# 86885974647565434342125458569795756674/torch.distributed.pipeline.sync.Pipe

Measured on AMD Instinct MI355X. Metric: tokens/sec for 12-layer Transformer at PP=N (pipeline-parallel training), higher is better.
Workload: dtype bf16

## Files before the change

mipipe/csrc/kernels/gemm.hip:

```cpp
#include <algorithm>
#include <cstdlib>

#include "common.h"
#include "kernels.h"

namespace mipipe {

namespace {

constexpr int BM = 128, BN = 128, BK = 64;
constexpr int kThreads = 256;
constexpr int kTileBytes = BM * BK * 2;
constexpr int kBufBytes = 2 * kTileBytes;
constexpr int kSmemBytes = 2 * kBufBytes;

typedef __attribute__((ext_vector_type(4))) short s16x4;
typedef __attribute__((ext_vector_type(8))) short s16x8;
typedef __attribute__((address_space(3))) s16x4 lds_s16x4;

__device__ __forceinline__ int kc_off(int r, int c16) { return r * 128 + ((c16 ^ ((r >> 1) & 7)) << 4); }

__device__ __forceinline__ int ic_rk(int r) { return (r & 3) | (((r >> 3) & 1) << 2); }
__device__ __forceinline__ int ic_off(int r, int c8) { return r * 256 + ((c8 ^ (ic_rk(r) << 2)) << 3); }

typedef __attribute__((ext_vector_type(4))) unsigned int u32x4;

template <bool KC>
struct Stager {
  u32x4 v[4];
  __device__ __forceinline__ void load(const bf16_t* __restrict__ base, int64_t ld, int i0, int k0, int tid) {
#pragma unroll
    for (int u = 0; u < 4; ++u) {
      const int id = tid + u * kThreads;
      const bf16_t* p;
      if (KC) {
        const int r = id >> 3, c = id & 7;
        p = base + (int64_t)(i0 + r) * ld + k0 + c * 8;
      } else {
        const int r = id >> 4, c = id & 15;
        p = base + (int64_t)(k0 + r) * ld + i0 + c * 8;
      }
      v[u] = *reinterpret_cast<const u32x4*>(p);
    }
  }
  __device__ __forceinline__ void store(char* tile, int tid) const {
#pragma unroll
    for (int u = 0; u < 4; ++u) {
      const int id = tid + u * kThreads;
      int off;
      if (KC) {
        off = kc_off(id >> 3, id & 7);
      } else {
        off = ic_off(id >> 4, (id & 15) * 2);
      }
      *reinterpret_cast<u32x4*>(tile + off) = v[u];
    }
  }
};

template <bool KC>
__device__ __forceinline__ bf16x8 read_frag(const char* tile, int ib, int s, int lane) {
  if (KC) {
    const int r = ib + (lane & 15);
    const int c = 4 * s + (lane >> 4);
    return *reinterpret_cast<const bf16x8*>(tile + kc_off(r, c));
  } else {
    const int g = lane >> 4, q = (lane & 15) >> 2, p = lane & 3;
    const int r0 = 32 * s + 8 * g + q;
    const int c8 = (ib >> 2) + p;
    const s16x4 lo = __builtin_amdgcn_ds_read_tr16_b64_v4i16((lds_s16x4*)(tile + ic_off(r0, c8)));
    const s16x4 hi = __builtin_amdgcn_ds_read_tr16_b64_v4i16((lds_s16x4*)(tile + ic_off(r0 + 4, c8)));
    const s16x8 both = __builtin_shufflevector(lo, hi, 0, 1, 2, 3, 4, 5, 6, 7);
    return __builtin_bit_cast(bf16x8, both);
  }
}

__device__ __forceinline__ float dact_f(int dact, float s) {
  return dact == kActRelu ? (s > 0.f ? 1.f : 0.f) : (dact == kActSavedGrad ? s : gelu_grad_f(s));
}

__device__ __forceinline__ void tile_coords(int tiles_m, int tiles_n, int& tm, int& tn, int G = 8) {
  const int nwg = tiles_m * tiles_n;
  const int bid = blockIdx.x;
  int wg = bid;
  if (nwg > 8) {
    const int xcd = bid & 7, local = bid >> 3;
    const int q = nwg >> 3, r = nwg & 7;
    wg = (xcd < r ? xcd * (q + 1) : r * (q + 1) + (xcd - r) * q) + local;
  }
  const int group = wg / (G * tiles_n);
  const int first_m = group * G;
  const int gsize = min(tiles_m - first_m, G);
  const int in_group = wg % (G * tiles_n);
  tm = first_m + in_group % gsize;
  tn = in_group / gsize;
}

template <bool A_KC, bool B_KC, int EPI, int ACT>
__global__ void __launch_bounds__(kThreads) gemm_kernel(GemmArgs g) {
  extern __shared__ __attribute__((aligned(16))) char smem[];
  const int tid = threadIdx.x;
  const int lane = tid & 63;
  const int wave = tid >> 6;
  const int wm = wave >> 1, wn = wave & 1;

  int tm, tn;
  tile_coords(g.M / BM, g.N / BN, tm, tn);
  const int m0 = tm * BM, n0 = tn * BN;

  const bf16_t* A = reinterpret_cast<const bf16_t*>(g.A);
  const bf16_t* B = reinterpret_cast<const bf16_t*>(g.B);

  f32x4 acc[4][4];
#pragma unroll
  for (int i = 0; i < 4; ++i)
#pragma unroll
    for (int j = 0; j < 4; ++j) acc[i][j] = f32x4{0.f, 0.f, 0.f, 0.f};

  Stager<A_KC> sa;
  Stager<B_KC> sb;
  const int nk = g.K / BK;

  sa.load(A, g.lda, m0, 0, tid);
  sb.load(B, g.ldb, n0, 0, tid);
  sa.store(smem, tid);
  sb.store(smem + kTileBytes, tid);
  __syncthreads();

  for (int kt = 0; kt < nk; ++kt) {
    char* cur = smem + (kt & 1) * kBufBytes;
    const bool more = kt + 1 < nk;
    if (more) {
      sa.load(A, g.lda, m0, (kt + 1) * BK, tid);
      sb.load(B, g.ldb, n0, (kt + 1) * BK, tid);
    }
#pragma unroll
    for (int s = 0; s < 2; ++s) {
      bf16x8 af[4], bfr[4];
#pragma unroll
      for (int t = 0; t < 4; ++t) af[t] = read_frag<A_KC>(cur, wm * 64 + 16 * t, s, lane);
#pragma unroll
      for (int t = 0; t < 4; ++t) bfr[t] = read_frag<B_KC>(cur + kTileBytes, wn * 64 + 16 * t, s, lane);
#pragma unroll
      for (int i = 0; i < 4; ++i)
#pragma unroll
        for (int j = 0; j < 4; ++j) acc[i][j] = __builtin_amdgcn_mfma_f32_16x16x32_bf16(af[i], bfr[j], acc[i][j], 0, 0, 0);
    }
    if (more) {
      char* nxt = smem + ((kt + 1) & 1) * kBufBytes;
      sa.store(nxt, tid);
      sb.store(nxt + kTileBytes, tid);
    }
    __syncthreads();
  }

  const int quad = lane >> 4, col_in = lane & 15;
  const float pscale = g.p > 0.f ? 1.f / (1.f - g.p) : 1.f;
#pragma unroll
  for (int i = 0; i < 4; ++i) {
    const int row0 = m0 + wm * 64 + 16 * i + 4 * quad;
#pragma unroll
    for (int j = 0; j < 4; ++j) {
      const int col = n0 + wn * 64 + 16 * j + col_in;
      f32x4 v = acc[i][j];
      if (EPI == kEpiAccumF32) {
        float* C = reinterpret_cast<float*>(g.C);
#pragma unroll
        for (int r = 0; r < 4; ++r) {
          float* p = C + (int64_t)(row0 + r) * g.ldc + col;
          *p += v[r];
        }
      } else if (EPI == kEpiStoreF32) {
        float* C = reinterpret_cast<float*>(g.C);
#pragma unroll
        for (int r = 0; r < 4; ++r) C[(int64_t)(row0 + r) * g.ldc + col] = v[r];
      } else {
        bf16_t* C = reinterpret_cast<bf16_t*>(g.C);
        const float b = g.bias != nullptr ? bf2f(reinterpret_cast<const bf16_t*>(g.bias)[col]) : 0.f;
        float pre[4], out[4];
#pragma unroll
        for (int r = 0; r < 4; ++r) {
          pre[r] = v[r] + b;
          out[r] = ACT == kActRelu ? fmaxf(pre[r], 0.f) : (ACT == kActGelu ? gelu_f(pre[r]) : pre[r]);
        }
        if (g.p > 0.f) {
          const uint4 w = Philox(g.seed, drop_sub(row0, col, g.N), g.offset).next4();
          const uint32_t ws[4] = {w.x, w.y, w.z, w.w};
#pragma unroll
          for (int r = 0; r < 4; ++r) out[r] = drop_keep(ws[r], col & 1, g.threshold >> 16) ? out[r] * pscale : 0.f;
        }
#pragma unroll
        for (int r = 0; r < 4; ++r) {
          if (g.dact_in != nullptr && g.dact == kActReluBits)
            out[r] *= (reinterpret_cast<const uint8_t*>(g.dact_in)[(int64_t)(row0 + r) * g.ldd + (col >> 3)] >> (col & 7)) & 1
                          ? g.dact_scale : 0.f;
          else if (g.dact_in != nullptr)
            out[r] *= g.dact_scale *
                      dact_f(g.dact, bf2f(reinterpret_cast<const bf16_t*>(g.dact_in)[(int64_t)(row0 + r) * g.ldd + col]));
          if (g.res != nullptr) out[r] += bf2f(reinterpret_cast<const bf16_t*>(g.res)[(int64_t)(row0 + r) * g.ldr + col]);
          C[(int64_t)(row0 + r) * g.ldc + col] = f2bf(out[r]);
          if (g.aux != nullptr)
            reinterpret_cast<bf16_t*>(g.aux)[(int64_t)(row0 + r) * g.ldc + col] =
                f2bf(g.aux_grad ? gelu_grad_f(pre[r]) : pre[r]);
        }
      }
    }
  }
}

namespace big {

constexpr int BM = 256, BN = 256, BK = 64;
constexpr int kThreads = 512;
constexpr int kTileBytes = BM * BK * 2;
constexpr int kSmemBytes = 128 * 260 * 4;

template <bool B_KC, int W>
constexpr int smem_bytes() {
  constexpr int b3 = 2 * (kTileBytes + W * BK * 2) + W * BK * 2;
  return !B_KC && b3 > kSmemBytes ? b3 : kSmemBytes;
}

template <int W>
__device__ __forceinline__ int ic_off_w(int r, int c8) { return r * (2 * W) + ((c8 ^ (ic_rk(r) << 2)) << 3); }

template <bool KC, int W>
__device__ __forceinline__ void stage_offsets(int64_t ld, int i0, int lim, int wave, int lane, uint32_t (&off)[W / 64]) {
  constexpr int NU = W / 64, LPR = W / 8;
#pragma unroll
  for (int u = 0; u < NU; ++u) {
    const int inst = wave * NU + u;
    if (KC) {
      const int row = 8 * inst + (lane >> 3);
      const int c = (lane & 7) ^ ((row >> 1) & 7);
      const int gi = min(i0 + row, lim - 1);
      off[u] = (uint32_t)(((int64_t)gi * ld + 8 * c) * 2);
    } else {
      const int row = (64 / LPR) * inst + lane / LPR;
      const int c16 = (lane % LPR) ^ (ic_rk(row) << 1);
      const int gi = min(i0 + 8 * c16, lim - 8);
      off[u] = (uint32_t)(((int64_t)row * ld + gi) * 2);
    }
  }
}

__device__ __forceinline__ void stage_offsets_halves(int64_t ld, int i0, int lim, int share, int lane,
                                                     uint32_t (&off)[4]) {
  const int half = share >> 2;
#pragma unroll
  for (int u = 0; u < 4; ++u) {
    const int row = 4 * (4 * (share & 3) + u) + (lane >> 4);
    const int c16 = (lane & 15) ^ (ic_rk(row) << 1);
    const int gi = min(i0 + 128 * half + 8 * c16, lim - 8);
    off[u] = (uint32_t)(((int64_t)row * ld + gi) * 2);
  }
}

__device__ __forceinline__ void glds16_saddr(const char* base, uint32_t off, const char* lds_dst) {
  const uint32_t m0 = (uint32_t)(uintptr_t)((__attribute__((address_space(3))) const char*)lds_dst);
  asm volatile(
      "s_mov_b32 m0, %0\n\t"
      "s_nop 0\n\t"
      "global_load_lds_dwordx4 %1, %2"
      :
      : "s"(m0), "v"(off), "s"(base)
      : "memory", "m0");
}

template <int N>
__device__ __forceinline__ void vmcnt_keep() {
  asm volatile("s_waitcnt vmcnt(%0)" ::"n"(N) : "memory");
}

constexpr int kWaitLgkm0 = 0xC07F;

template <int W>
__device__ __forceinline__ void stage_fast(const char* base, const uint32_t (&off)[W / 64], char* tile, int wave) {
  constexpr int NU = W / 64;
#pragma unroll
  for (int u = 0; u < NU; ++u) glds16_saddr(base, off[u], tile + (wave * NU + u) * 1024);
}

struct KCursor {
  const char *a, *b;
  const char *na, *nb;
  int64_t step_a, step_b;
  int seg_k, kl, seg;

  __device__ __forceinline__ void load_next(const GemmArgs& g) {
    const int nx = min(seg + 1, GemmArgs::kMaxSegs - 1);
    na = reinterpret_cast<const char*>(g.a_seg[nx]);
    nb = reinterpret_cast<const char*>(g.b_seg[nx]);
  }
  template <bool A_KC, bool B_KC>
  __device__ __forceinline__ void init(const GemmArgs& g, int kt) {
    const int64_t lda = g.lda, ldb = g.ldb;
    step_a = A_KC ? BK * 2 : BK * lda * 2;
    step_b = B_KC ? BK * 2 : BK * ldb * 2;
    seg_k = g.seg_k;
    kl = kt * BK;
    seg = 0;
    a = na = reinterpret_cast<const char*>(g.A);
    b = nb = reinterpret_cast<const char*>(g.B);
    if (seg_k > 0) {
      seg = kl / seg_k;
      kl -= seg * seg_k;
      a = reinterpret_cast<const char*>(g.a_seg[seg]);
      b = reinterpret_cast<const char*>(g.b_seg[seg]);
      load_next(g);
    }
    a += A_KC ? (int64_t)kl * 2 : (int64_t)kl * lda * 2;
    b += B_KC ? (int64_t)kl * 2 : (int64_t)kl * ldb * 2;
  }
  __device__ __forceinline__ void next(const GemmArgs& g) {
    a += step_a;
    b += step_b;
    kl += BK;
    if (__builtin_expect(kl == seg_k, 0)) {
      kl = 0;
      ++seg;
      a = na;
      b = nb;
      load_next(g);
    }
  }
};

template <bool KC, int W>
__device__ __forceinline__ bf16x8 frag(const char* tile, int ib, int s, int lane) {
  if (KC) {
    const int r = ib + (lane & 15);
    const int c = 4 * s + (lane >> 4);
    return *reinterpret_cast<const bf16x8*>(tile + kc_off(r, c));
  } else {
    const int g = lane >> 4, q = (lane & 15) >> 2, p = lane & 3;
    const int r0 = 32 * s + 8 * g + q;
    const int c8 = (ib >> 2) + p;
    const s16x4 lo = __builtin_amdgcn_ds_read_tr16_b64_v4i16((lds_s16x4*)(tile + ic_off_w<W>(r0, c8)));
    const s16x4 hi = __builtin_amdgcn_ds_read_tr16_b64_v4i16((lds_s16x4*)(tile + ic_off_w<W>(r0 + 4, c8)));
    return __builtin_bit_cast(bf16x8, __builtin_shufflevector(lo, hi, 0, 1, 2, 3, 4, 5, 6, 7));
  }
}

struct EpiParams {
  uint64_t seed, offset;
  int N;
  float p, pscale;
  uint32_t threshold;
  int mask_row0, mask_col0, mask_ld;
};

template <int I, int ACT, int NJ, bool EXTRA>
__device__ __forceinline__ void epi_rows(const EpiParams ep, f32x4 (&acc)[8][NJ], int nrow, int ncol,
                                         const float (&bias)[NJ]) {
  if constexpr (!EXTRA) {
#pragma unroll
    for (int j = 0; j < NJ; ++j)
#pragma unroll
      for (int r = 0; r < 4; ++r) {
        const float pre = acc[I][j][r] + bias[j];
        acc[I][j][r] = ACT == kActRelu ? fmaxf(pre, 0.f) : (ACT == kActGelu ? gelu_f(pre) : pre);
      }
    return;
  }
  const int row0 = nrow + 16 * I;
#pragma unroll
  for (int j = 0; j < NJ; ++j) {
    const int col = ncol + 16 * j;
    const float b = bias[j];
    uint32_t ws[4] = {0xFFFFFFFFu, 0xFFFFFFFFu, 0xFFFFFFFFu, 0xFFFFFFFFu};
    if (ep.p > 0.f) {
      const uint4 w = Philox(ep.seed, drop_sub(row0 + ep.mask_row0, col + ep.mask_col0, ep.mask_ld), ep.offset).next4();
      ws[0] = w.x; ws[1] = w.y; ws[2] = w.z; ws[3] = w.w;
    }
#pragma unroll
    for (int r = 0; r < 4; ++r) {
      const float pre = acc[I][j][r] + b;
      float out = ACT == kActRelu ? fmaxf(pre, 0.f) : (ACT == kActGelu ? gelu_f(pre) : pre);
      if (ep.p > 0.f) out = drop_keep(ws[r], (col + ep.mask_col0) & 1, ep.threshold >> 16) ? out * ep.pscale : 0.f;
      acc[I][j][r] = out;
    }
  }
}

template <int EPI, int W>
__device__ __forceinline__ void staged_store(char* smem, const f32x4 (&acc)[8][W / 64], int wm, int wn, int lane,
                                             int tid, int m0, int n0, int M, int N, int64_t ldc, void* out,
                                             const bf16_t* res, int64_t ldr = 0, const bf16_t* dact_in = nullptr,
                                             int64_t ldd = 0, int dact = 0, float dact_scale = 1.f,
                                             bool trans = false, bool dgelu = false) {
  constexpr int NJ = W / 64, WN = 16 * NJ, kStride = W + 4;
  const int quad = lane >> 4, col_in = lane & 15;
  float* stg = reinterpret_cast<float*>(smem);
#pragma unroll
  for (int pass = 0; pass < 2; ++pass) {
    if (wm == pass) {
#pragma unroll
      for (int i = 0; i < 8; ++i)
#pragma unroll
        for (int j = 0; j < NJ; ++j)
#pragma unroll
          for (int r = 0; r < 4; ++r)
            stg[(16 * i + 4 * quad + r) * kStride + wn * WN + 16 * j + col_in] = acc[i][j][r];
    }
    __syncthreads();
    const int rbase = m0 + pass * 128;
    auto grow = [&](int R) { return rbase + R; };
    if (EPI == kEpiStoreBf16) {
      bf16_t* C = reinterpret_cast<bf16_t*>(out);
      constexpr int CPR = W / 8;
#pragma unroll
      for (int u = 0; u < 128 * CPR / kThreads; ++u) {
        const int idx = tid + u * kThreads;
        const int row = idx / CPR, c8 = idx % CPR;
        if (grow(row) >= M || n0 + 8 * c8 >= N) continue;
        const f32x4 lo = *reinterpret_cast<const f32x4*>(stg + row * kStride + 8 * c8);
        const f32x4 hi = *reinterpret_cast<const f32x4*>(stg + row * kStride + 8 * c8 + 4);
        const int64_t at = (int64_t)grow(row) * ldc + n0 + 8 * c8;
        float v[8] = {lo[0], lo[1], lo[2], lo[3], hi[0], hi[1], hi[2], hi[3]};
        if (dgelu) {
#pragma unroll
          for (int e = 0; e < 8; ++e) v[e] = gelu_grad_f(v[e]);
        }
        if (dact_in != nullptr && dact == kActReluBits) {
          const uint32_t mb =
              reinterpret_cast<const uint8_t*>(dact_in)[(int64_t)grow(row) * ldd + ((n0 + 8 * c8) >> 3)];
#pragma unroll
          for (int e = 0; e < 8; ++e) v[e] *= (mb >> e) & 1 ? dact_scale : 0.f;
        } else if (dact_in != nullptr) {
          const bf16x8 sv = *reinterpret_cast<const bf16x8*>(dact_in + (int64_t)grow(row) * ldd + n0 + 8 * c8);
#pragma unroll
          for (int e = 0; e < 8; ++e) v[e] *= dact_scale * dact_f(dact, (float)sv[e]);
        }
        if (res != nullptr) {
          const bf16x8 rv = *reinterpret_cast<const bf16x8*>(res + (int64_t)grow(row) * ldr + n0 + 8 * c8);
#pragma unroll
          for (int e = 0; e < 8; ++e) v[e] += (float)rv[e];
        }
        bf16x8 o;
#pragma unroll
        for (int e = 0; e < 8; ++e) o[e] = (__bf16)v[e];
        *reinterpret_cast<bf16x8*>(C + at) = o;
      }
    } else if (trans) {
      float* C = reinterpret_cast<float*>(out);
#pragma unroll 4
      for (int u = 0; u < 32 * W / kThreads; ++u) {
        const int idx = tid + u * kThreads;
        const int mq = (idx & 7) + 8 * (idx / (8 * W)), n = (idx >> 3) % W;
        if (grow(4 * mq) >= M || n0 + n >= N) continue;
        const float* sp = stg + 4 * mq * kStride + n;
        const float4 v = make_float4(sp[0], sp[kStride], sp[2 * kStride], sp[3 * kStride]);
        float4* dst = reinterpret_cast<float4*>(C + (int64_t)(n0 + n) * ldc + grow(4 * mq));
        if (EPI == kEpiAccumF32) {
          const float4 o = *dst;
          *dst = make_float4(o.x + v.x, o.y + v.y, o.z + v.z, o.w + v.w);
        } else {
          *dst = v;
        }
      }
    } else {
      float* C = reinterpret_cast<float*>(out);
      constexpr int CPR = W / 4;
#pragma unroll
      for (int u = 0; u < 128 * CPR / kThreads; ++u) {
        const int idx = tid + u * kThreads;
        const int row = idx / CPR, c4 = idx % CPR;
        if (grow(row) >= M || n0 + 4 * c4 >= N) continue;
        const float4 v = *reinterpret_cast<const float4*>(stg + row * kStride + 4 * c4);
        float4* dst = reinterpret_cast<float4*>(C + (int64_t)grow(row) * ldc + n0 + 4 * c4);
        if (EPI == kEpiAccumF32) {
          const float4 o = *dst;
          *dst = make_float4(o.x + v.x, o.y + v.y, o.z + v.z, o.w + v.w);
        } else {
          *dst = v;
        }
      }
    }
    __syncthreads();
  }
}

template <int ACT, int W>
__device__ __forceinline__ void staged_store_act(char* smem, const f32x4 (&acc)[8][W / 64], int wm, int wn,
                                                 int lane, int tid, int m0, int n0, const GemmArgs& g) {
  constexpr int NJ = W / 64, WN = 16 * NJ, kStride = W + 4, CB = W / 8;
  const int quad = lane >> 4, col_in = lane & 15;
  float* stg = reinterpret_cast<float*>(smem);
  bf16_t* C = reinterpret_cast<bf16_t*>(g.C);
  bf16_t* aux = reinterpret_cast<bf16_t*>(g.aux);
  const bf16_t* res = reinterpret_cast<const bf16_t*>(g.res);
  const bf16_t* dact_in = reinterpret_cast<const bf16_t*>(g.dact_in);
  const int64_t ldr = g.ldr > 0 ? g.ldr : g.ldc;
  const bool drop = g.p > 0.f;
  const float pscale = drop ? 1.f / (1.f - g.p) : 1.f;
  const int64_t mask_ld = g.mask_ld > 0 ? g.mask_ld : g.N;
  const uint32_t thr16 = g.threshold >> 16;
#pragma unroll
  for (int pass = 0; pass < 2; ++pass) {
    if (wm == pass) {
#pragma unroll
      for (int i = 0; i < 8; ++i)
#pragma unroll
        for (int j = 0; j < NJ; ++j)
#pragma unroll
          for (int r = 0; r < 4; ++r)
            stg[(16 * i + 4 * quad + r) * kStride + wn * WN + 16 * j + col_in] = acc[i][j][r];
    }
    __syncthreads();
    const int rbase = m0 + pass * 128;
#pragma unroll
    for (int u = 0; u < 32 * CB / kThreads; ++u) {
      const int idx = tid + u * kThreads;
      const int rq = idx / CB, c8 = idx % CB;
      const int col = n0 + 8 * c8;
      const int row0 = rbase + 4 * rq;
      if (col >= g.N || row0 >= g.M) continue;
      uint32_t wd[4][4];
      if (drop) {
        const uint64_t sub = drop_sub(row0 + g.mask_row0, col + g.mask_col0, mask_ld);
#pragma unroll
        for (int e = 0; e < 4; ++e) {
          const uint4 w = Philox(g.seed, sub + e, g.offset).next4();
          wd[e][0] = w.x; wd[e][1] = w.y; wd[e][2] = w.z; wd[e][3] = w.w;
        }
      }
#pragma unroll
      for (int r = 0; r < 4; ++r) {
        const int row = row0 + r;
        if (row >= g.M) break;
        const float* sp = stg + (4 * rq + r) * kStride + 8 * c8;
        const f32x4 lo = *reinterpret_cast<const f32x4*>(sp);
        const f32x4 hi = *reinterpret_cast<const f32x4*>(sp + 4);
        const float pre[8] = {lo[0], lo[1], lo[2], lo[3], hi[0], hi[1], hi[2], hi[3]};
        if (aux != nullptr) {
          bf16x8 a;
#pragma unroll
          for (int e = 0; e < 8; ++e) a[e] = (__bf16)(ACT == kActGelu && g.aux_grad ? gelu_grad_f(pre[e]) : pre[e]);
          *reinterpret_cast<bf16x8*>(aux + (int64_t)row * g.ldc + col) = a;
        }
        float v[8];
#pragma unroll
        for (int e = 0; e < 8; ++e) {
          float o = ACT == kActRelu ? fmaxf(pre[e], 0.f) : (ACT == kActGelu ? gelu_f(pre[e]) : pre[e]);
          if (drop) o = drop_keep(wd[e >> 1][r], e & 1, thr16) ? o * pscale : 0.f;
          v[e] = o;
        }
        if (dact_in != nullptr) {
          const bf16x8 sv = *reinterpret_cast<const bf16x8*>(dact_in + (int64_t)row * g.ldd + col);
#pragma unroll
          for (int e = 0; e < 8; ++e) v[e] *= g.dact_scale * dact_f(g.dact, (float)sv[e]);
        }
        if (res != nullptr) {
          const bf16x8 rv = *reinterpret_cast<const bf16x8*>(res + (int64_t)row * ldr + col);
#pragma unroll
          for (int e = 0; e < 8; ++e) v[e] += (float)rv[e];
        }
        bf16x8 o;
#pragma unroll
        for (int e = 0; e < 8; ++e) o[e] = (__bf16)v[e];
        *reinterpret_cast<bf16x8*>(C + (int64_t)row * g.ldc + col) = o;
        if (g.bits != nullptr) {
          uint32_t mb = 0;
#pragma unroll
          for (int e = 0; e < 8; ++e) mb |= (v[e] != 0.f ? 1u : 0u) << e;
          reinterpret_cast<uint8_t*>(g.bits)[(int64_t)row * g.ldbits + (col >> 3)] = (uint8_t)mb;
        }
      }
    }
    __syncthreads();
  }
}


constexpr int kXEmit = 1, kXColsum = 2;

template <bool A_KC, bool B_KC, int EPI, int ACT, int W, bool EXTRA, int X = 0>
__global__ void __launch_bounds__(kThreads, 1) gemm256_kernel(GemmArgs g) {
  constexpr int NJ = W / 64;
  constexpr int WN = W / 4;
  constexpr int kBuf = kTileBytes + W * BK * 2;
  constexpr bool AH = !A_KC;
  constexpr bool B3 = !B_KC;
  extern __shared__ __attribute__((aligned(16))) char smem[];
  const int tid = threadIdx.x;
  const int lane = tid & 63;
  const int wave = __builtin_amdgcn_readfirstlane(tid >> 6);
  const int wm = wave >> 2, wn = wave & 3;

  int tm, tn;
  tile_coords((g.M + BM - 1) / BM, (g.N + W - 1) / W, tm, tn, g.group_m);
  tm = __builtin_amdgcn_readfirstlane(tm);
  tn = __builtin_amdgcn_readfirstlane(tn);
  const int m0 = tm * BM, n0 = tn * W;
  f32x4 acc[8][NJ];
#pragma unroll
  for (int i = 0; i < 8; ++i)
#pragma unroll
    for (int j = 0; j < NJ; ++j) acc[i][j] = f32x4{0.f, 0.f, 0.f, 0.f};

  const bool rsum = g.rowsum != nullptr && tn < 16 && !A_KC;
  float rs[4] = {0.f, 0.f, 0.f, 0.f};
  auto rowsum_read = [&](const char* tile, s16x4& v) {
    if (rsum && wm == 0) {
      const int r = tid >> 2, c8 = 4 * tn + (tid & 3);
      v = *reinterpret_cast<const s16x4*>(
          AH ? tile + (tn >> 3) * (kTileBytes / 2) + ic_off_w<128>(r, c8 & 31) : tile + ic_off_w<256>(r, c8));
    }
  };
  auto rowsum_add = [&](const s16x4& v) {
    if (rsum && wm == 0) {
#pragma unroll
      for (int e = 0; e < 4; ++e) rs[e] += __uint_as_float((uint32_t)(uint16_t)v[e] << 16);
    }
  };
  const int tiles_m = (g.M + BM - 1) / BM;
  const int cm_log = __builtin_amdgcn_readfirstlane(2 * tiles_m * 16 >= W ? 0 : 2 * tiles_m * 32 >= W ? 1
                                                    : 2 * tiles_m * 64 >= W ? 2 : 3);
  const int csl = tm + tiles_m * wm;
  const bool csum = X == kXColsum && !B_KC && g.colsum != nullptr && csl < (W / 16 >> cm_log);
  float cs[4] = {0.f, 0.f, 0.f, 0.f};
  auto colsum_step = [&](const char* btile) {
    if (csum) {
      const int t = tid & 255;
      const int q = t & ((4 << cm_log) - 1), r0 = t >> (2 + cm_log);
      for (int j = 0; j < (1 << cm_log); ++j) {
        const s16x4 v = *reinterpret_cast<const s16x4*>(
            btile + ic_off_w<W>(r0 + (j << (6 - cm_log)), (4 << cm_log) * csl + q));
#pragma unroll
        for (int e = 0; e < 4; ++e) cs[e] += __uint_as_float((uint32_t)(uint16_t)v[e] << 16);
      }
    }
  };
  const int ntn = (g.N + W - 1) / W;
  const int ewb = __builtin_amdgcn_readfirstlane((4 * wave) % ntn);
  auto emit_reads = [&](const char* atile, int j, s16x4& a, s16x4& b) {
    const int q = (lane & 15) >> 2, p = lane & 3, gq = lane >> 4;
    const int c16 = 2 * gq + (p >> 1);
    const int r = 8 * (4 * wave + j) + q;
    const int lo = r * 128 + ((c16 ^ ((r >> 1) & 7)) << 4) + 8 * (p & 1);
    const int hi = (r + 4) * 128 + ((c16 ^ (((r + 4) >> 1) & 7)) << 4) + 8 * (p & 1);
    a = __builtin_amdgcn_ds_read_tr16_b64_v4i16((lds_s16x4*)(atile + lo));
    b = __builtin_amdgcn_ds_read_tr16_b64_v4i16((lds_s16x4*)(atile + hi));
  };
  bf16_t* const at_out = X == kXEmit ? reinterpret_cast<bf16_t*>(g.at) : nullptr;
  const int64_t ldat = X == kXEmit ? g.ldat : 0;
  const int M = g.M;
  auto emit_store = [&](int kt, int j, const s16x4& a, const s16x4& b) {
    const int rb = 4 * wave + j;
    bf16_t* at = at_out + (int64_t)(kt * BK + 16 * (lane >> 4) + (lane & 15)) * ldat + m0 + 8 * rb;
    if (m0 + 8 * rb < M) *reinterpret_cast<s16x8*>(at) = __builtin_shufflevector(a, b, 0, 1, 2, 3, 4, 5, 6, 7);
  };
  int kt0 = 0, nk = g.K / BK;
  if (g.k_splits > 1) {
    const int total = nk;
    kt0 = (int)blockIdx.y * total / g.k_splits;
    nk = ((int)blockIdx.y + 1) * total / g.k_splits - kt0;
  }
  const int shA = wave ^ 4;
  const int shB = B_KC ? 2 * wn + (wm == 0 ? 1 : 0) : wave;
  uint32_t offA[4], offB[NJ];
  if constexpr (AH) stage_offsets_halves(g.lda, m0, g.M, shA, lane, offA);
  else stage_offsets<A_KC, 256>(g.lda, m0, g.M, shA, lane, offA);
  stage_offsets<B_KC, W>(g.ldb, n0, g.N, shB, lane, offB);
  constexpr int NB = W / 64;
  constexpr int NA = 4;
  KCursor kc;
  kc.init<A_KC, B_KC>(g, kt0);
  stage_fast<256>(kc.a, offA, smem, shA);
  stage_fast<W>(kc.b, offB, smem + kTileBytes, shB);
  kc.next(g);
  if (wm == 1 && nk > 1) {
    stage_fast<256>(kc.a, offA, smem + kBuf, shA);
    stage_fast<W>(kc.b, offB, smem + kBuf + kTileBytes, shB);
    kc.next(g);
  }

  if (wm == 1 && nk > 1) vmcnt_keep<NA + NB>();
  else asm volatile("s_waitcnt vmcnt(0)" ::: "memory");
  __builtin_amdgcn_s_barrier();
  if (wm == 1) __builtin_amdgcn_s_barrier();
  bf16x8 af[8][2], bq[NJ][2];
  int ekt = kt0 % ntn;
  auto bslot = [&](int s) { return s == 2 ? smem + 2 * kBuf : smem + s * kBuf + kTileBytes; };
  int bs = 0;
  for (int u = 0; u < nk; ++u) {
    char* cur = smem + (u & 1) * kBuf;
    char* nxt = smem + ((u + 1) & 1) * kBuf;
    char* bcur = B3 ? bslot(bs) : cur + kTileBytes;
    int ej = -1;
    if (X == kXEmit && A_KC) {
      int e = ewb + ekt;
      while (e >= ntn) e -= ntn;
      ej = tn - e;
      if (ej < 0) ej += ntn;
      if (ntn < 4) {
        for (int j = ej; j < 4; j += ntn) {
          s16x4 a, b;
          emit_reads(cur, j, a, b);
          emit_store(kt0 + u, j, a, b);
        }
        ej = -1;
      } else if (ej > 3) {
        ej = -1;
      }
    }
    s16x4 ea, eb;
    if (X == kXEmit && A_KC && ej >= 0) emit_reads(cur, ej, ea, eb);
#pragma unroll
    for (int ii = 0; ii < 8; ++ii)
#pragma unroll
      for (int s = 0; s < 2; ++s)
        af[ii][s] = AH ? frag<false, 128>(cur + wm * (kTileBytes / 2), 16 * ii, s, lane)
                       : frag<A_KC, 256>(cur, wm * 128 + 16 * ii, s, lane);
#pragma unroll
    for (int j = 0; j < NJ; ++j)
#pragma unroll
      for (int s = 0; s < 2; ++s) bq[j][s] = frag<B_KC, W>(bcur, wn * WN + 16 * j, s, lane);
    s16x4 rv;
    rowsum_read(cur, rv);
    if (X == kXEmit && A_KC && ej >= 0) emit_store(kt0 + u, ej, ea, eb);
    ekt = ekt + 1 == ntn ? 0 : ekt + 1;
    const int ahead = wm == 0 ? 1 : 2;
    if (u + ahead < nk) {
      char* dst = wm == 0 ? nxt : cur;
      stage_fast<256>(kc.a, offA, dst, shA);
      int bn = bs + ahead;
      if (bn >= 3) bn -= 3;
      stage_fast<W>(kc.b, offB, B3 ? bslot(bn) : dst + kTileBytes, shB);
      kc.next(g);
    }
    bs = bs == 2 ? 0 : bs + 1;
    colsum_step(bcur);
    if (wm == 1) {
      if (u + 2 < nk) vmcnt_keep<NA + NB>();
      else asm volatile("s_waitcnt vmcnt(0)" ::: "memory");
    }
    __builtin_amdgcn_s_waitcnt(kWaitLgkm0);
    rowsum_add(rv);
    __builtin_amdgcn_sched_barrier(0);
    __builtin_amdgcn_s_barrier();
    __builtin_amdgcn_sched_barrier(0);
    __builtin_amdgcn_s_setprio(1);
#pragma unroll
    for (int s = 0; s < 2; ++s)
#pragma unroll
      for (int ii = 0; ii < 8; ++ii)
#pragma unroll
        for (int j = 0; j < NJ; ++j)
          acc[ii][j] = __builtin_amdgcn_mfma_f32_16x16x32_bf16(af[ii][s], bq[j][s], acc[ii][j], 0, 0, 0);
    __builtin_amdgcn_s_setprio(0);
    if (wm == 0) asm volatile("s_waitcnt vmcnt(0)" ::: "memory");
    __builtin_amdgcn_sched_barrier(0);
    __builtin_amdgcn_s_barrier();
    __builtin_amdgcn_sched_barrier(0);
  }
  if (wm == 0) __builtin_amdgcn_s_barrier();

  if (rsum) {
    __syncthreads();
    float* red = reinterpret_cast<float*>(smem);
    if (wm == 0) {
#pragma unroll
      for (int e = 0; e < 4; ++e)
#pragma unroll
        for (int o = 4; o < 64; o <<= 1) rs[e] += __shfl_xor(rs[e], o, 64);
      if (lane < 4)
#pragma unroll
        for (int e = 0; e < 4; ++e) red[wave * 16 + 4 * lane + e] = rs[e];
    }
    __syncthreads();
    if (tid < 16) {
      const float v = red[tid] + red[16 + tid] + red[32 + tid] + red[48 + tid];
      const int row = m0 + 16 * tn + tid;
      if (row < g.M) g.rowsum[row] += v;
    }
  }
  if (X == kXColsum && g.colsum != nullptr) {
    __syncthreads();
    const int sw = 16 << cm_log;
    float* red = reinterpret_cast<float*>(smem) + 64;
#pragma unroll
    for (int e = 0; e < 4; ++e)
      for (int o = 4 << cm_log; o < 64; o <<= 1) cs[e] += __shfl_xor(cs[e], o, 64);
    if (lane < (4 << cm_log))
#pragma unroll
      for (int e = 0; e < 4; ++e) red[wave * sw + 4 * lane + e] = cs[e];
    __syncthreads();
    if (tid < 2 * sw) {
      const int gq = tid >> (4 + cm_log), c = tid & (sw - 1);
      const int sl = tm + tiles_m * gq;
      float v = 0.f;
#pragma unroll
      for (int w = 0; w < 4; ++w) v += red[(4 * gq + w) * sw + c];
      const int col = n0 + sw * sl + c;
      if (sl < (W / 16 >> cm_log) && col < g.N) {
        if (g.k_splits > 1) g.colsum[(int64_t)blockIdx.y * g.N + col] = v;
        else g.colsum[col] += v;
      }
    }
  }
  const int quad = lane >> 4, col_in = lane & 15;
  __syncthreads();
  if (EPI == kEpiStoreBf16 && EXTRA) {
    const int ncol = n0 + wn * WN + col_in;
    if (g.bias != nullptr) {
#pragma unroll
      for (int j = 0; j < NJ; ++j) {
        const float b = ncol + 16 * j < g.N ? bf2f(reinterpret_cast<const bf16_t*>(g.bias)[ncol + 16 * j]) : 0.f;
#pragma unroll
        for (int i = 0; i < 8; ++i) acc[i][j] += b;
      }
    }
    staged_store_act<ACT, W>(smem, acc, wm, wn, lane, tid, m0, n0, g);
    return;
  }
  if (EPI == kEpiStoreBf16 && (ACT != kActNone || g.bias != nullptr)) {
    const int ncol = n0 + wn * WN + col_in, nrow = m0 + wm * 128 + 4 * quad;
    const float pscale = g.p > 0.f ? 1.f / (1.f - g.p) : 1.f;
    const EpiParams ep{g.seed, g.offset, g.N, g.p, pscale, g.threshold, g.mask_row0, g.mask_col0,
                       g.mask_ld > 0 ? g.mask_ld : g.N};
    float bias[NJ];
#pragma unroll
    for (int j = 0; j < NJ; ++j)
      bias[j] = (g.bias != nullptr && ncol + 16 * j < g.N) ? bf2f(reinterpret_cast<const bf16_t*>(g.bias)[ncol + 16 * j]) : 0.f;
    epi_rows<0, ACT, NJ, EXTRA>(ep, acc, nrow, ncol, bias);
    epi_rows<1, ACT, NJ, EXTRA>(ep, acc, nrow, ncol, bias);
    epi_rows<2, ACT, NJ, EXTRA>(ep, acc, nrow, ncol, bias);
    epi_rows<3, ACT, NJ, EXTRA>(ep, acc, nrow, ncol, bias);
    epi_rows<4, ACT, NJ, EXTRA>(ep, acc, nrow, ncol, bias);
    epi_rows<5, ACT, NJ, EXTRA>(ep, acc, nrow, ncol, bias);
    epi_rows<6, ACT, NJ, EXTRA>(ep, acc, nrow, ncol, bias);
    epi_rows<7, ACT, NJ, EXTRA>(ep, acc, nrow, ncol, bias);
  }
  void* out = EPI == kEpiStoreBf16 ? g.C
                                   : reinterpret_cast<void*>(reinterpret_cast<float*>(g.C) +
                                                             (int64_t)blockIdx.y * g.M * g.ldc);
  if (EPI == kEpiStoreBf16 && g.dact_in != nullptr)
    staged_store<EPI, W>(smem, acc, wm, wn, lane, tid, m0, n0, g.M, g.N, g.ldc, out,
                         reinterpret_cast<const bf16_t*>(g.res), g.ldr, reinterpret_cast<const bf16_t*>(g.dact_in),
                         g.ldd, g.dact, g.dact_scale);
  else if (EPI != kEpiStoreBf16 && g.trans_c && g.k_splits <= 1)
    staged_store<EPI, W>(smem, acc, wm, wn, lane, tid, m0, n0, g.M, g.N, g.ldc, out, nullptr, 0, nullptr, 0, 0, 1.f,
                         true);
  else
    staged_store<EPI, W>(smem, acc, wm, wn, lane, tid, m0, n0, g.M, g.N, g.ldc, out,
                         EPI == kEpiStoreBf16 ? reinterpret_cast<const bf16_t*>(g.res) : nullptr, g.ldr);
}

}

int big_tiles(const GemmArgs& g, int w) { return ((g.M + big::BM - 1) / big::BM) * ((g.N + w - 1) / w); }

bool use_big(const GemmArgs& g) {
  return g.round_chunk || g.seg_k > 0 || g.at != nullptr || g.trans_c || g.colsum != nullptr || g.rowsum != nullptr ||
         g.M % BM != 0 || g.N % BN != 0 || big_tiles(g, 256) >= 128;
}

int g_gemm_width = -1;
int g_gemm_rounds = -1;

int big_width(const GemmArgs& g) {
  if (g_gemm_width < 0) {
    const char* e = getenv("MIPIPE_GEMM_W");
    g_gemm_width = e ? atoi(e) : 0;
  }
  if (g_gemm_width == 128 || g_gemm_width == 256) return g_gemm_width;
  if (g.width == 128 || g.width == 256) return g.width;
  if (g.k_splits > 1) return 256;
  const int r256 = (big_tiles(g, 256) + 255) / 256, r128 = (big_tiles(g, 128) + 255) / 256;
  return 0.75 * r128 < 1.0 * r256 ? 128 : 256;
}

template <bool A_KC, bool B_KC, int EPI, int ACT, int W, bool EXTRA, int X = 0>
void launch_big(const GemmArgs& g, hipStream_t s) {
  constexpr int smem = big::smem_bytes<B_KC, W>();
  static bool attr_set = false;
  if (!attr_set) {
    (void)hipFuncSetAttribute(
        reinterpret_cast<const void*>(&big::gemm256_kernel<A_KC, B_KC, EPI, ACT, W, EXTRA, X>),
        hipFuncAttributeMaxDynamicSharedMemorySize, smem);
    attr_set = true;
  }
  hipLaunchKernelGGL((big::gemm256_kernel<A_KC, B_KC, EPI, ACT, W, EXTRA, X>), dim3(big_tiles(g, W), g.k_splits),
                     dim3(big::kThreads), smem, s, g);
}

template <bool A_KC, bool B_KC, int EPI, int ACT, bool EXTRA>
void launch_big_w(const GemmArgs& g, hipStream_t s) {
  const bool narrow = big_width(g) == 128;
  if constexpr (A_KC && B_KC && EPI == kEpiStoreBf16 && !(ACT == kActGelu && EXTRA)) {
    if (g.at != nullptr) {
      if (narrow) launch_big<A_KC, B_KC, EPI, ACT, 128, EXTRA, big::kXEmit>(g, s);
      else launch_big<A_KC, B_KC, EPI, ACT, 256, EXTRA, big::kXEmit>(g, s);
      return;
    }
  }
  if constexpr (A_KC && !B_KC && EPI != kEpiStoreBf16 && !EXTRA) {
    if (g.colsum != nullptr) {
      if (narrow) launch_big<A_KC, B_KC, EPI, ACT, 128, EXTRA, big::kXColsum>(g, s);
      else launch_big<A_KC, B_KC, EPI, ACT, 256, EXTRA, big::kXColsum>(g, s);
      return;
    }
  }
  if (narrow) launch_big<A_KC, B_KC, EPI, ACT, 128, EXTRA>(g, s);
  else launch_big<A_KC, B_KC, EPI, ACT, 256, EXTRA>(g, s);
}

int g_gemm_group = -1;

template <bool A_KC, bool B_KC, int EPI, int ACT>
void launch(const GemmArgs& gi, hipStream_t s) {
  if (g_gemm_group < 0) {
    const char* e = getenv("MIPIPE_GEMM_G");
    g_gemm_group = e ? atoi(e) : 0;
  }
  GemmArgs g = gi;
  if (g_gemm_group > 0) g.group_m = g_gemm_group;
  if (use_big(g)) {
    if constexpr (EPI == kEpiStoreBf16) {
      if (g.p > 0.f || g.aux != nullptr) {
        launch_big_w<A_KC, B_KC, EPI, ACT, true>(g, s);
        return;
      }
    }
    launch_big_w<A_KC, B_KC, EPI, ACT, false>(g, s);
    return;
  }
  const int blocks = (g.M / BM) * (g.N / BN);
  hipLaunchKernelGGL((gemm_kernel<A_KC, B_KC, EPI, ACT>), dim3(blocks), dim3(kThreads), kSmemBytes, s, g);
}

__global__ void __launch_bounds__(256) splitk_reduce_kernel(const float* __restrict__ ws, int splits, int M, int N,
                                                            int64_t ldc, const bf16_t* __restrict__ res, int64_t ldr,
                                                            bf16_t* __restrict__ C) {
  const int64_t chunks = (int64_t)M * (N / 8);
  const int64_t c = (int64_t)blockIdx.x * blockDim.x + threadIdx.x;
  if (c >= chunks) return;
  const int row = (int)(c / (N / 8)), col = (int)(c % (N / 8)) * 8;
  const int64_t at = (int64_t)row * N + col;
  f32x4 lo = *reinterpret_cast<const f32x4*>(ws + at);
  f32x4 hi = *reinterpret_cast<const f32x4*>(ws + at + 4);
  for (int s = 1; s < splits; ++s) {
    lo += *reinterpret_cast<const f32x4*>(ws + (int64_t)s * M * N + at);
    hi += *reinterpret_cast<const f32x4*>(ws + (int64_t)s * M * N + at + 4);
  }
  float v[8] = {lo[0], lo[1], lo[2], lo[3], hi[0], hi[1], hi[2], hi[3]};
  const int64_t out = (int64_t)row * ldc + col;
  if (res != nullptr) {
    const bf16x8 r = *reinterpret_cast<const bf16x8*>(res + (int64_t)row * ldr + col);
#pragma unroll
    for (int e = 0; e < 8; ++e) v[e] += (float)r[e];
  }
  bf16x8 o;
#pragma unroll
  for (int e = 0; e < 8; ++e) o[e] = (__bf16)v[e];
  *reinterpret_cast<bf16x8*>(C + out) = o;
}

__global__ void __launch_bounds__(256) splitk_reduce_f32_kernel(const float* __restrict__ ws, int splits, int M, int N,
                                                                int64_t ldc, bool accumulate, bool trans,
                                                                float* __restrict__ C) {
  const int64_t c = (int64_t)blockIdx.x * blockDim.x + threadIdx.x;
  if (trans) {
    if (c >= (int64_t)(M / 4) * N) return;
    const int m = (int)(c / N) * 4, n = (int)(c % N);
    f32x4 v = {0.f, 0.f, 0.f, 0.f};
    for (int s = 0; s < splits; ++s) {
      const float* p = ws + (int64_t)s * M * N + (int64_t)m * N + n;
      v += f32x4{p[0], p[N], p[2 * (int64_t)N], p[3 * (int64_t)N]};
    }
    f32x4* dst = reinterpret_cast<f32x4*>(C + (int64_t)n * ldc + m);
    if (accumulate) v += *dst;
    *dst = v;
    return;
  }
  const int64_t chunks = (int64_t)M * (N / 4);
  if (c >= chunks) return;
  const int row = (int)(c / (N / 4)), col = (int)(c % (N / 4)) * 4;
  const int64_t at = (int64_t)row * N + col;
  f32x4 v = *reinterpret_cast<const f32x4*>(ws + at);
  for (int s = 1; s < splits; ++s) v += *reinterpret_cast<const f32x4*>(ws + (int64_t)s * M * N + at);
  f32x4* dst = reinterpret_cast<f32x4*>(C + (int64_t)row * ldc + col);
  if (accumulate) v += *dst;
  *dst = v;
}

__global__ void __launch_bounds__(256) colsum_splits_kernel(const float* __restrict__ ws, int splits, int N,
                                                            float* __restrict__ colsum) {
  const int n = blockIdx.x * blockDim.x + threadIdx.x;
  if (n >= N) return;
  float v = 0.f;
  for (int s = 0; s < splits; ++s) v += ws[(int64_t)s * N + n];
  colsum[n] += v;
}

int g_gemm_splitk = -1;

template <bool A_KC, bool B_KC, int EPI>
void launch_act(const GemmArgs& g, hipStream_t s) {
  switch (g.act) {
    case kActRelu: launch<A_KC, B_KC, EPI, kActRelu>(g, s); break;
    case kActGelu: launch<A_KC, B_KC, EPI, kActGelu>(g, s); break;
    default: launch<A_KC, B_KC, EPI, kActNone>(g, s); break;
  }
}

}

void gemm_set_width(int w) { g_gemm_width = w; }
void gemm_set_rounds(int on) { g_gemm_rounds = on; }
void gemm_set_splitk(int n) { g_gemm_splitk = n; }

bool gemm_rowsum_ok(const GemmArgs& g) {
  return !g.a_kc && (g.epi == kEpiAccumF32 || g.epi == kEpiStoreF32) && use_big(g) && gemm_splitk_factor(g) <= 1 &&
         (g.N + big_width(g) - 1) / big_width(g) >= 16;
}

bool gemm_bits_ok(const GemmArgs& g) {
  return g.epi == kEpiStoreBf16 && g.act == kActRelu && g.p > 0.f && g.k_splits <= 1 && g.N % 8 == 0 && use_big(g);
}

bool gemm_emit_ok(int act, float p, bool aux) { return !(act == kActGelu && (p > 0.f || aux)); }

bool gemm_colsum_ok(const GemmArgs& g) {
  if (g.b_kc || !g.a_kc || !(g.epi == kEpiAccumF32 || g.epi == kEpiStoreF32)) return false;
  GemmArgs b = g;
  b.k_splits = gemm_splitk_factor(g);
  const int w = big_width(b);
  return 2 * ((g.M + big::BM - 1) / big::BM) * 128 >= w;
}

bool gemm_supported(int64_t M, int64_t N, int64_t K) {
  return M >= 8 && N >= 8 && K > 0 && M % 8 == 0 && N % 8 == 0 && K % BK == 0 && M < (1LL << 30) &&
         N < (1LL << 30) && M * K < (1LL << 31) && N * K < (1LL << 31);
}

int gemm_splitk_factor(const GemmArgs& g) {
  if (g_gemm_splitk < 0) {
    const char* e = getenv("MIPIPE_GEMM_SPLITK");
    g_gemm_splitk = e ? atoi(e) : 1;
  }
  if (g_gemm_splitk == 0) return 1;
  const bool plain_bf16 = g.epi == kEpiStoreBf16 && g.act == kActNone && g.bias == nullptr && g.p <= 0.f &&
                          g.aux == nullptr && g.dact_in == nullptr;
  const bool f32_out = g.epi == kEpiAccumF32 || g.epi == kEpiStoreF32;
  if (!(plain_bf16 || f32_out) || !use_big(g) || g.K < 8192) return 1;
  const int tiles = big_tiles(g, 256);
  const int kt = g.K / BK;
  if (g_gemm_splitk >= 2) return std::max(1, std::min(g_gemm_splitk, kt / 16));
  const double t_tile = 2.0 * 256 * 256 * (double)g.K / 4.5e12;
  const double mn = (double)g.M * g.N;
  int best = 1;
  double best_t = (double)((tiles + 255) / 256) * t_tile;
  for (int sp = 2; sp <= 8 && kt / sp >= 16; ++sp) {
    const double t = (double)((tiles * sp + 255) / 256) * t_tile / sp + (2.0 * sp + 1.0) * 4.0 * mn / 4.0e12;
    if (t < 0.97 * best_t) {
      best = sp;
      best_t = t;
    }
  }
  return best;
}


static const char* byte_off(const void* p, int64_t bytes) {
  return p == nullptr ? nullptr : reinterpret_cast<const char*>(p) + bytes;
}

template <typename F>
bool launch_by_rounds(const GemmArgs& g, F&& run) {
  if (g_gemm_rounds < 0) {
    const char* e = getenv("MIPIPE_GEMM_ROUNDS");
    g_gemm_rounds = e ? atoi(e) : 1;
  }
  if (g_gemm_rounds == 0 || g.k_splits > 1 || !use_big(g) || big_width(g) != 256) return false;
  if (g_gemm_rounds == 1 && g.K < 4096) return false;
  const int tm = (g.M + 255) / 256, tn = (g.N + 255) / 256;
  if (tm * tn <= 256 || (tm * tn) % 256 == 0 || (tm * tn) % 256 > 128) return false;
  const bool along_n = tn >= tm;
  if (along_n && g.rowsum != nullptr) return false;
  if (!along_n && g.colsum != nullptr) return false;
  const int other = along_n ? tm : tn, along = along_n ? tn : tm;
  const int per = 256 / other;
  if (per < 1 || (along + per - 1) / per > 16) return false;
  const int cbytes = g.epi == kEpiStoreBf16 ? 2 : 4;
  for (int t0 = 0; t0 < along; t0 += per) {
    GemmArgs c = g;
    c.round_chunk = true;
    c.width = 256;
    const int lo = t0 * 256, hi = std::min((t0 + per) * 256, along_n ? g.N : g.M);
    c.mask_ld = g.mask_ld > 0 ? g.mask_ld : g.N;
    if (along_n) {
      c.N = hi - lo;
      c.mask_col0 = g.mask_col0 + lo;
      const int64_t boff = (g.b_kc ? (int64_t)lo * g.ldb : (int64_t)lo) * 2;
      c.B = byte_off(g.B, boff);
      for (int i = 0; i < GemmArgs::kMaxSegs; ++i) c.b_seg[i] = byte_off(g.b_seg[i], boff);
      c.C = const_cast<char*>(byte_off(g.C, (g.trans_c ? (int64_t)lo * g.ldc : (int64_t)lo) * cbytes));
      if (g.colsum != nullptr) c.colsum = g.colsum + lo;
      if (t0 > 0) c.at = nullptr;
      c.bias = byte_off(g.bias, (int64_t)lo * 2);
      c.aux = const_cast<char*>(byte_off(g.aux, (int64_t)lo * 2));
      c.res = byte_off(g.res, (int64_t)lo * 2);
      c.dact_in = byte_off(g.dact_in, g.dact == kActReluBits ? (int64_t)lo / 8 : (int64_t)lo * 2);
      c.bits = const_cast<char*>(byte_off(g.bits, (int64_t)lo / 8));
    } else {
      c.M = hi - lo;
      c.mask_row0 = g.mask_row0 + lo;
      if (g.rowsum != nullptr) c.rowsum = g.rowsum + lo;
      const int64_t aoff = (g.a_kc ? (int64_t)lo * g.lda : (int64_t)lo) * 2;
      c.A = byte_off(g.A, aoff);
      for (int i = 0; i < GemmArgs::kMaxSegs; ++i) c.a_seg[i] = byte_off(g.a_seg[i], aoff);
      c.C = const_cast<char*>(byte_off(g.C, (g.trans_c ? (int64_t)lo : (int64_t)lo * g.ldc) * cbytes));
      c.at = const_cast<char*>(byte_off(g.at, (int64_t)lo * 2));
      c.aux = const_cast<char*>(byte_off(g.aux, (int64_t)lo * g.ldc * 2));
      c.res = byte_off(g.res, (int64_t)lo * g.ldr * 2);
      c.dact_in = byte_off(g.dact_in, (int64_t)lo * g.ldd * (g.dact == kActReluBits ? 1 : 2));
      c.bits = const_cast<char*>(byte_off(g.bits, (int64_t)lo * g.ldbits));
    }
    run(c);
  }
  return true;
}

void gemm_bf16(const GemmArgs& gi, hipStream_t s) {
  GemmArgs g = gi;
  g.threshold = dropout_threshold(g.p);
  if (g.ldr == 0) g.ldr = g.ldc;
  if (g.ldd == 0) g.ldd = g.ldc;
  if (g.k_splits > 1) {
    GemmArgs p = g;
    p.epi = kEpiStoreF32;
    p.C = g.ws;
    p.ldc = g.N;
    p.res = nullptr;
    p.trans_c = false;
    p.rowsum = nullptr;
    p.colsum = g.colsum != nullptr ? g.colsum_ws : nullptr;
    if (p.a_kc && p.b_kc) launch<true, true, kEpiStoreF32, kActNone>(p, s);
    else if (p.a_kc && !p.b_kc) launch<true, false, kEpiStoreF32, kActNone>(p, s);
    else if (!p.a_kc && !p.b_kc) launch<false, false, kEpiStoreF32, kActNone>(p, s);
    else launch<false, true, kEpiStoreF32, kActNone>(p, s);
    if (g.epi == kEpiStoreBf16) {
      const int64_t chunks = (int64_t)g.M * (g.N / 8);
      hipLaunchKernelGGL(splitk_reduce_kernel, dim3((unsigned)((chunks + 255) / 256)), dim3(256), 0, s, g.ws,
                         g.k_splits, g.M, g.N, g.ldc, reinterpret_cast<const bf16_t*>(g.res), g.ldr,
                         reinterpret_cast<bf16_t*>(g.C));
    } else {
      const int64_t chunks = (int64_t)g.M * (g.N / 4);
      hipLaunchKernelGGL(splitk_reduce_f32_kernel, dim3((unsigned)((chunks + 255) / 256)), dim3(256), 0, s, g.ws,
                         g.k_splits, g.M, g.N, g.ldc, g.epi == kEpiAccumF32, g.trans_c,
                         reinterpret_cast<float*>(g.C));
      if (g.colsum != nullptr)
        hipLaunchKernelGGL(colsum_splits_kernel, dim3((unsigned)((g.N + 255) / 256)), dim3(256), 0, s, g.colsum_ws,
                           g.k_splits, g.N, g.colsum);
    }
    return;
  }
  auto dispatch = [s](const GemmArgs& g) {
    if (g.epi == kEpiStoreBf16) {
      if (g.a_kc && g.b_kc) launch_act<true, true, kEpiStoreBf16>(g, s);
      else if (g.a_kc && !g.b_kc) launch_act<true, false, kEpiStoreBf16>(g, s);
      else if (!g.a_kc && !g.b_kc) launch_act<false, false, kEpiStoreBf16>(g, s);
      else launch_act<false, true, kEpiStoreBf16>(g, s);
    } else if (g.epi == kEpiAccumF32) {
      if (g.a_kc && g.b_kc) launch<true, true, kEpiAccumF32, kActNone>(g, s);
      else if (g.a_kc && !g.b_kc) launch<true, false, kEpiAccumF32, kActNone>(g, s);
      else if (!g.a_kc && !g.b_kc) launch<false, false, kEpiAccumF32, kActNone>(g, s);
      else launch<false, true, kEpiAccumF32, kActNone>(g, s);
    } else {
      if (g.a_kc && g.b_kc) launch<true, true, kEpiStoreF32, kActNone>(g, s);
      else if (g.a_kc && !g.b_kc) launch<true, false, kEpiStoreF32, kActNone>(g, s);
      else if (!g.a_kc && !g.b_kc) launch<false, false, kEpiStoreF32, kActNone>(g, s);
      else launch<false, true, kEpiStoreF32, kActNone>(g, s);
    }
  };
  if (!launch_by_rounds(g, dispatch)) dispatch(g);
}

}
```

Before: 155,300.

## Add specialized K-loop for transposed-A and transposed-B GEMM with precomputed LDS addresses

For the case where both A and B are stored non-K-contiguous, the kernel gets its own main loop. It uses a new LDS layout: two A buffers back to back, followed by three B slots. LDS fragment addresses are computed once per lane and then used with constant offsets, and the loop is unrolled by two so buffer parity is known at compile time. The goal is to remove per-iteration address arithmetic and to make the transposed LDS reads (ds_read_tr) cheaper in the inner loop. The cost is more code and a separate path whose synchronization must match the generic loop.

Result: faster. 157,200 (median of 6 runs) (+1.2%).

```diff
diff --git a/mipipe/csrc/kernels/gemm.hip b/mipipe/csrc/kernels/gemm.hip
--- a/mipipe/csrc/kernels/gemm.hip
+++ b/mipipe/csrc/kernels/gemm.hip
@@ -1,5 +1,6 @@
 #include <algorithm>
 #include <cstdlib>
+#include <type_traits>
 
 #include "common.h"
 #include "kernels.h"
@@ -342,6 +343,20 @@
   }
 }
 
+template <int W>
+__device__ __forceinline__ uint32_t ic_frag_off(int ib, int lane) {
+  const int g = lane >> 4, q = (lane & 15) >> 2, p = lane & 3;
+  return (uint32_t)ic_off_w<W>(8 * g + q, (ib >> 2) + p);
+}
+
+template <int W>
+__device__ __forceinline__ bf16x8 ic_frag_at(uint32_t addr, int imm, int s) {
+  const s16x4 lo = __builtin_amdgcn_ds_read_tr16_b64_v4i16((lds_s16x4*)(addr + (uint32_t)(imm + s * 32 * 2 * W)));
+  const s16x4 hi =
+      __builtin_amdgcn_ds_read_tr16_b64_v4i16((lds_s16x4*)(addr + (uint32_t)(imm + s * 32 * 2 * W + 4 * 2 * W)));
+  return __builtin_bit_cast(bf16x8, __builtin_shufflevector(lo, hi, 0, 1, 2, 3, 4, 5, 6, 7));
+}
+
 struct EpiParams {
   uint64_t seed, offset;
   int N;
@@ -582,6 +597,7 @@
   constexpr int kBuf = kTileBytes + W * BK * 2;
   constexpr bool AH = !A_KC;
   constexpr bool B3 = !B_KC;
+  constexpr bool II = AH && B3;
   extern __shared__ __attribute__((aligned(16))) char smem[];
   const int tid = threadIdx.x;
   const int lane = tid & 63;
@@ -665,14 +681,19 @@
   stage_offsets<B_KC, W>(g.ldb, n0, g.N, shB, lane, offB);
   constexpr int NB = W / 64;
   constexpr int NA = 4;
+  auto abuf = [&](int i) { return II ? smem + i * kTileBytes : smem + i * kBuf; };
+  auto bslot = [&](int s) {
+    if (II) return smem + 2 * kTileBytes + s * (W * BK * 2);
+    return s == 2 ? smem + 2 * kBuf : smem + s * kBuf + kTileBytes;
+  };
   KCursor kc;
   kc.init<A_KC, B_KC>(g, kt0);
-  stage_fast<256>(kc.a, offA, smem, shA);
-  stage_fast<W>(kc.b, offB, smem + kTileBytes, shB);
+  stage_fast<256>(kc.a, offA, abuf(0), shA);
+  stage_fast<W>(kc.b, offB, bslot(0), shB);
   kc.next(g);
   if (wm == 1 && nk > 1) {
-    stage_fast<256>(kc.a, offA, smem + kBuf, shA);
-    stage_fast<W>(kc.b, offB, smem + kBuf + kTileBytes, shB);
+    stage_fast<256>(kc.a, offA, abuf(1), shA);
+    stage_fast<W>(kc.b, offB, bslot(1), shB);
     kc.next(g);
   }
 
@@ -682,9 +703,70 @@
   if (wm == 1) __builtin_amdgcn_s_barrier();
   bf16x8 af[8][2], bq[NJ][2];
   int ekt = kt0 % ntn;
-  auto bslot = [&](int s) { return s == 2 ? smem + 2 * kBuf : smem + s * kBuf + kTileBytes; };
   int bs = 0;
-  for (int u = 0; u < nk; ++u) {
+  if constexpr (II) {
+    const uint32_t lds0 = (uint32_t)(uintptr_t)((__attribute__((address_space(3))) const char*)smem);
+    uint32_t aaddr[8], baddr[NJ];
+#pragma unroll
+    for (int ii = 0; ii < 8; ++ii) aaddr[ii] = lds0 + wm * (kTileBytes / 2) + ic_frag_off<128>(16 * ii, lane);
+#pragma unroll
+    for (int j = 0; j < NJ; ++j) baddr[j] = ic_frag_off<W>(wn * WN + 16 * j, lane);
+    auto k_tile = [&](const int u, auto parity) {
+      constexpr int P = decltype(parity)::value;
+      char* cur = abuf(P);
+      char* nxt = abuf(P ^ 1);
+      char* bcur = bslot(bs);
+#pragma unroll
+      for (int ii = 0; ii < 8; ++ii)
+#pragma unroll
+        for (int s = 0; s < 2; ++s) af[ii][s] = ic_frag_at<128>(aaddr[ii], P * kTileBytes, s);
+      const uint32_t bcur0 = (uint32_t)(uintptr_t)((__attribute__((address_space(3))) const char*)bcur);
+#pragma unroll
+      for (int j = 0; j < NJ; ++j) {
+        const uint32_t ba = bcur0 + baddr[j];
+#pragma unroll
+        for (int s = 0; s < 2; ++s) bq[j][s] = ic_frag_at<W>(ba, 0, s);
+      }
+      s16x4 rv;
+      rowsum_read(cur, rv);
+      const int ahead = wm == 0 ? 1 : 2;
+      if (u + ahead < nk) {
+        stage_fast<256>(kc.a, offA, wm == 0 ? nxt : cur, shA);
+        int bn = bs + ahead;
+        if (bn >= 3) bn -= 3;
+        stage_fast<W>(kc.b, offB, bslot(bn), shB);
+        kc.next(g);
+      }
+      bs = bs == 2 ? 0 : bs + 1;
+      if (wm == 1) {
+        if (u + 2 < nk) vmcnt_keep<NA + NB>();
+        else asm volatile("s_waitcnt vmcnt(0)" ::: "memory");
+      }
+      __builtin_amdgcn_s_waitcnt(kWaitLgkm0);
+      rowsum_add(rv);
+      __builtin_amdgcn_sched_barrier(0);
+      __builtin_amdgcn_s_barrier();
+      __builtin_amdgcn_sched_barrier(0);
+      __builtin_amdgcn_s_setprio(1);
+#pragma unroll
+      for (int s = 0; s < 2; ++s)
+#pragma unroll
+        for (int ii = 0; ii < 8; ++ii)
+#pragma unroll
+          for (int j = 0; j < NJ; ++j)
+            acc[ii][j] = __builtin_amdgcn_mfma_f32_16x16x32_bf16(af[ii][s], bq[j][s], acc[ii][j], 0, 0, 0);
+      __builtin_amdgcn_s_setprio(0);
+      if (wm == 0) asm volatile("s_waitcnt vmcnt(0)" ::: "memory");
+      __builtin_amdgcn_sched_barrier(0);
+      __builtin_amdgcn_s_barrier();
+      __builtin_amdgcn_sched_barrier(0);
+    };
+    for (int u = 0; u < nk; u += 2) {
+      k_tile(u, std::integral_constant<int, 0>{});
+      if (u + 1 < nk) k_tile(u + 1, std::integral_constant<int, 1>{});
+    }
+  }
+  for (int u = 0; !II && u < nk; ++u) {
     char* cur = smem + (u & 1) * kBuf;
     char* nxt = smem + ((u + 1) & 1) * kBuf;
     char* bcur = B3 ? bslot(bs) : cur + kTileBytes;
```
